# wzx99/DCFP

Measured on AMD Instinct MI355X. Metric: training images/sec at 1024x2048 DeepLabv3-R101, higher is better.
Workload: dtype f32

## Files before the change

dcfp_amd/csrc/conv_igemm.hip:

```cpp
#include "common.h"
#include <string.h>
#include <stdio.h>
#include <stdlib.h>

namespace {

int check_desc(const DcfpConvDesc* d) {
    if (!d) return DCFP_E_BADDESC;
    if (d->N <= 0 || d->Cin <= 0 || d->Cout <= 0 || d->H <= 0 || d->W <= 0 || d->stride <= 0 ||
        d->dil <= 0 || d->pad < 0)
        return DCFP_E_BADDESC;
    if (d->KH != d->KW || (d->KH != 1 && d->KH != 3)) return DCFP_E_UNSUPPORTED;
    const int ho = (d->H + 2 * d->pad - d->dil * (d->KH - 1) - 1) / d->stride + 1;
    const int wo = (d->W + 2 * d->pad - d->dil * (d->KW - 1) - 1) / d->stride + 1;
    if (ho != d->Hout || wo != d->Wout || ho <= 0 || wo <= 0) return DCFP_E_BADDESC;
    if ((d->x_pitch != 0 && (d->x_pitch < d->W || (d->x_pitch & 3))) ||
        (d->dy_pitch != 0 && (d->dy_pitch < d->Wout || (d->dy_pitch & 3))))
        return DCFP_E_BADDESC;
    if ((long long)d->Cin * d->H * (d->x_pitch ? d->x_pitch : d->W) >= (1LL << 29) ||
        (long long)d->Cout * d->Hout * (d->dy_pitch ? d->dy_pitch : d->Wout) >= (1LL << 29) ||
        (long long)d->Cout * d->Cin * d->KH * d->KW >= (1LL << 29))
        return DCFP_E_UNSUPPORTED;
    return DCFP_OK;
}
// ... 12 lines not shown
                    const float* bias, float* out, long long out_nstride, int N, int M, int Ck, int T,
                    int Hi, int Wi, int Ho, int Wo, int sn, int sd, int off0, int offstep,
                    int accumulate, void* workspace, size_t workspace_bytes, hipStream_t stream,
                    const float* scale = nullptr, const float* shift = nullptr,
                    const float* residual = nullptr, int relu = 0, float* stat_part = nullptr, int wp_valid = 0,
                    int in_pitch = 0, long long wp_nstride = 0, const float* fan_src = nullptr,
                    const unsigned long long* fan_mask = nullptr, const Igemm2Red* red = nullptr);
bool dcfp_wino_ok(int N, int H, int W, int d, int M, int Ck);
size_t dcfp_wino_workspace_bytes(int N, int H, int W, int d, int M, int Ck);
double dcfp_wino_exec_fraction(int N, int H, int W, int d, int M, int Ck);
int dcfp_wino_run(const float* in, long long in_nstride, int in_pitch, const float* w, int sAm, int sAc, int flip,
                  float* out, long long out_nstride, int N, int M, int Ck, int H, int W, int d, int accumulate,
                  void* workspace, size_t workspace_bytes, hipStream_t stream, float* xform_out = nullptr,
                  float* stat_part = nullptr, const float* scale = nullptr, const float* shift = nullptr,
                  const float* residual = nullptr, int relu = 0, int wp_valid = 0);
long long dcfp_wino_stat_slots(int N, int H, int W, int d);
bool dcfp_stem_shape(const DcfpConvDesc* d);
int dcfp_stem_fwd(const DcfpConvDesc* d, const float* x, const float* w, const float* bias, float* y, long long y_nstride,
                  hipStream_t stream, float* stat_part = nullptr);
long long dcfp_stem_stat_slots(const DcfpConvDesc* d, const float* y, long long y_nstride);
bool dcfp_gemv_shape(const DcfpConvDesc* d);
int dcfp_gemv_fwd(const DcfpConvDesc* d, const float* x, const float* w, const float* bias, float* y, long long y_nstride,
                  hipStream_t stream);
int dcfp_gemv_dgrad(const DcfpConvDesc* d, const float* dy, long long dy_nstride, const float* w, float* dx, int accumulate,
                    hipStream_t stream);
bool dcfp_wino_fused_ok(int N, int H, int W, int d, int M, int Ck, long long in_nstride, int pitch);
size_t dcfp_wino_fused_workspace_bytes(int N, int H, int W, int d, int M, int Ck);
void dcfp_wino_fused_pads(int N, int H, int W, int d, int M, int Ck, int* CkP, int* Mpad);
size_t dcfp_wino_xform_bytes(int N, int H, int W, int d, int C);
bool dcfp_wgrad_is_winograd(const DcfpConvDesc* d);
bool dcfp_wgrad_wants_xform(const DcfpConvDesc* d);
long long dcfp_igemm2_stat_slots(int M, int P, int N, long long out_nstride, const float* out);
bool dcfp_igemm2_dma_shape(int T, int M, int Ck, int P, long long px, int sn, int sd, int off0, int HiWi, int Wo);
bool dcfp_igemm2_persist();
void dcfp_igemm2_wp_layout(int T, int M, int Ck, int P, long long px, int sn, int sd, int off0, int offstep, int HiWi,
                           int Wo, bool pitched, int sAm, int sAc, DcfpWpEntry* e);
bool dcfp_igemm2_use_dma8(int T, int M, int P, long long px, int sn, int sd, int off0, int offstep, int HiWi,
                          int Wo, bool pitched);
int dcfp_igemm2_permute_multi(const DcfpWpEntry* table, int n, long long total_blocks, hipStream_t stream);


size_t dcfp_igemm3_workspace_bytes(int T, int M, int Ck);
int dcfp_igemm3_run(const float* in, long long in_nstride, const float* w, int sAm, int sAc,
                    const float* bias, float* out, long long out_nstride, int N, int M, int Ck, int T,
                    int Hi, int Wi, int Ho, int Wo, int off0, int offstep, int accumulate,
                    void* workspace, size_t workspace_bytes, hipStream_t stream,
                    const float* scale = nullptr, const float* shift = nullptr,
                    const float* residual = nullptr, int relu = 0, int wp_valid = 0);
int dcfp_igemm2_cfg_id(int M, long long px, int sd);
static bool math_bf16x3() {
    static const bool v = [] { const char* e = getenv("DCFP_CONV_MATH"); return e && !strcmp(e, "bf16x3"); }();
    return v;
}
static bool igemm3_ok(int M, long long px, int sn, int sd) {
    return math_bf16x3() && sn == 1 && sd == 1 && dcfp_igemm2_cfg_id(M, px, sd) == 4;
}

static int wino_kind(const DcfpConvDesc* d, int pass) {
    static const int mode = [] { const char* e = getenv("DCFP_CONV_WINOGRAD"); return e ? atoi(e) : 1; }();
    if (mode == 0) return 0;
    if (d->KH != 3 || d->KW != 3 || d->stride != 1 || d->pad != d->dil || d->Hout != d->H || d->Wout != d->W)
        return 0;
    if (math_bf16x3()) return 0;
    const bool fwd = pass == DCFP_CONV_FWD;
    const int M = fwd ? d->Cout : d->Cin, Ck = fwd ? d->Cin : d->Cout;
    const int sp = fwd ? d->x_pitch : d->dy_pitch;
// ... 66 lines not shown
        const long long px = (long long)d->N * d->H * d->W;
        b2 = dcfp_igemm2_workspace_bytes(T, d->Cin, d->Cout, px, d->stride);
        if (igemm3_ok(d->Cin, px, 1, d->stride)) b3 = dcfp_igemm3_workspace_bytes(T, d->Cin, d->Cout);
    }
    return b2 > b3 ? b2 : b3;
}

extern "C" int dcfp_conv2d_kernel_name(const DcfpConvDesc* d, int pass, char* buf, int buf_len) {
    int rc = check_desc(d);
    if (rc) return rc;
    if (!buf || buf_len <= 0) return DCFP_E_BADDESC;
    if (dcfp_gemv_shape(d)) return snprintf(buf, buf_len, "gemv_1x1_map_kernel");
    if (pass == DCFP_CONV_WGRAD) return dcfp_wgrad_kernel_name(d, buf, buf_len);
    if (pass == DCFP_CONV_FWD && dcfp_stem_shape(d)) return snprintf(buf, buf_len, "stem_fwd_kernel");
    if (const int wk = wino_kind(d, pass))
        return wk == 1 ? snprintf(buf, buf_len, "winograd_f2x2_3x3 (igemm2_dma1p_kernel<false,true>)")
                       : snprintf(buf, buf_len, "winograd_f2x2_3x3 fused (wino_fused_kernel)");
    const int M = pass == DCFP_CONV_FWD ? d->Cout : d->Cin;
    const long long px = pass == DCFP_CONV_FWD ? (long long)d->N * d->Hout * d->Wout : (long long)d->N * d->H * d->W;
    const int sd = pass == DCFP_CONV_FWD ? 1 : d->stride;
    if (igemm3_ok(M, px, pass == DCFP_CONV_FWD ? d->stride : 1, sd))
        return snprintf(buf, buf_len, "igemm3_kernel<%d>", d->KH * d->KW);
    const int P = pass == DCFP_CONV_FWD ? d->Hout * d->Wout : d->H * d->W;
    const int HiWi = pass == DCFP_CONV_FWD ? d->H * d->W : d->Hout * d->Wout;
    const int Ck = pass == DCFP_CONV_FWD ? d->Cin : d->Cout;
    {
        const int sp = pass == DCFP_CONV_FWD ? d->x_pitch : d->dy_pitch;
        const bool pitched = sp && sp != (pass == DCFP_CONV_FWD ? d->W : d->Wout);
        if (dcfp_igemm2_use_dma8(d->KH * d->KW, M, P, px, pass == DCFP_CONV_FWD ? d->stride : 1, sd,
                                 pass == DCFP_CONV_FWD ? -d->pad : d->pad, pass == DCFP_CONV_FWD ? d->dil : -d->dil,
                                 HiWi, pass == DCFP_CONV_FWD ? d->Wout : d->W, pitched))
            return snprintf(buf, buf_len, "igemm2_dma8_kernel<%d>", d->KH * d->KW);
    }
    if (dcfp_igemm2_dma_shape(d->KH * d->KW, M, Ck, P, px, pass == DCFP_CONV_FWD ? d->stride : 1, sd, d->pad, HiWi,
                              pass == DCFP_CONV_FWD ? d->Wout : d->W)) {
        if (d->KH == 1 && dcfp_igemm2_persist()) return snprintf(buf, buf_len, "igemm2_dma1p_kernel");
        const int src_pitch = pass == DCFP_CONV_FWD ? d->x_pitch : d->dy_pitch;
        const bool pitched = src_pitch && src_pitch != (pass == DCFP_CONV_FWD ? d->W : d->Wout);
        return snprintf(buf, buf_len, "igemm2_dma_kernel<%d,%s>", d->KH * d->KW,
                        (d->KH == 3 && ((d->pad | d->dil) & 3) != 0 && !pitched) ? "true" : "false");
    }
    return snprintf(buf, buf_len, "igemm2_kernel<%d,%s>", d->KH * d->KW, dcfp_igemm2_cfg_args(M, px, sd));
}

extern "C" double dcfp_conv2d_executed_fraction(const DcfpConvDesc* d, int pass) {
    if (check_desc(d) != DCFP_OK) return 1.0;
    if (pass == DCFP_CONV_WGRAD) return dcfp_wgrad_exec_fraction(d);
    const bool fwd = pass == DCFP_CONV_FWD;
    if (wino_pass(d, pass))
        return fwd ? dcfp_wino_exec_fraction(d->N, d->H, d->W, d->dil, d->Cout, d->Cin)
                   : dcfp_wino_exec_fraction(d->N, d->H, d->W, d->dil, d->Cin, d->Cout);
    const int M = fwd ? d->Cout : d->Cin;
    const long long px = fwd ? (long long)d->N * d->Hout * d->Wout : (long long)d->N * d->H * d->W;
    if (igemm3_ok(M, px, fwd ? d->stride : 1, fwd ? 1 : d->stride)) return 1.0;
    const int sp = fwd ? d->x_pitch : d->dy_pitch;
    const bool pitched = sp && sp != (fwd ? d->W : d->Wout);
    return fwd ? dcfp_igemm2_exec_fraction(d->KH * d->KW, d->Cout, d->Cin, d->N, d->H, d->W, d->Hout, d->Wout, d->stride, 1,
                                           -d->pad, d->dil, pitched)
               : dcfp_igemm2_exec_fraction(d->KH * d->KW, d->Cin, d->Cout, d->N, d->Hout, d->Wout, d->H, d->W, 1, d->stride,
                                           d->pad, -d->dil, pitched);
}

extern "C" int64_t dcfp_conv2d_fwd_stat_slots(const DcfpConvDesc* d, const float* y, int64_t y_nstride);

extern "C" size_t dcfp_conv2d_xform_bytes(const DcfpConvDesc* d) {
    if (check_desc(d) != DCFP_OK) return 0;
// ... 240 lines not shown
```

dcfp_amd/csrc/conv_igemm2.hip:

```cpp
#include "igemm2_common.h"
#include <queue>
#include <vector>
#include <stdio.h>
#include <stdlib.h>

namespace {

__device__ __forceinline__ int wp_row(int m, int perm8) {
    if (!perm8) return m;
    const int j = m & 255;
    return (m & ~255) + 32 * (j & 7) + (j >> 3);
}

__global__ void __launch_bounds__(256)
permute_weights_kernel(const float* __restrict__ w, float* __restrict__ wp, int T, int Ck, int CkP,
                       int M, int Mpad, int sAm, int sAc, int perm8) {
    const long long total = (long long)T * CkP * Mpad;
    for (long long i = (long long)blockIdx.x * 256 + threadIdx.x; i < total;
         i += (long long)gridDim.x * 256) {
        const int m = wp_row((int)(i % Mpad), perm8);
        const long long r = i / Mpad;
        const int c = (int)(r % CkP);
        const int t = (int)(r / CkP);
        float v = 0.f;
// ... 5 lines not shown
constexpr int kWpBlockElems = DCFP_WP_BLOCK_ELEMS;
__global__ void __launch_bounds__(256)
permute_weights_multi_kernel(const DcfpWpEntry* __restrict__ table, int n) {
    const long long blk = blockIdx.x;
    int lo = 0, hi = n - 1;
    while (lo < hi) {
        const int mid = (lo + hi + 1) >> 1;
        if (table[mid].first_block <= blk) lo = mid; else hi = mid - 1;
    }
    const DcfpWpEntry e = table[lo];
    const long long base = (blk - e.first_block) * kWpBlockElems;
    if (e.perm8 >= 2) {
        const long long pairs = (long long)e.CkP * e.Mpad;
#pragma unroll 1
        for (int u = 0; u < kWpBlockElems / 256; ++u) {
            const long long i = base + u * 256 + threadIdx.x;
            if (i >= pairs) return;
            wino_filter2_pair(e.w, e.sAm, e.sAc, e.perm8 == 3, e.M, e.Ck, e.Mpad, i, e.wp);
        }
        return;
    }
    const long long total = (long long)e.T * e.CkP * e.Mpad;
#pragma unroll
    for (int u = 0; u < kWpBlockElems / 256; ++u) {
        const long long i = base + u * 256 + threadIdx.x;
        if (i >= total) return;
        const int m = wp_row((int)(i % e.Mpad), e.perm8);
        const long long r = i / e.Mpad;
        const int c = (int)(r % e.CkP);
        const int t = (int)(r / e.CkP);
        float v = 0.f;
        if (m < e.M && c < e.Ck) v = e.w[(long long)m * e.sAm + (long long)c * e.sAc + t];
        e.wp[i] = v;
    }
}

__device__ __forceinline__ float half_xor(float v, int mask) {
    switch (mask) {
        case 1: return __builtin_bit_cast(float, __builtin_amdgcn_ds_swizzle(__builtin_bit_cast(int, v), (1 << 10) | 0x1f));
        case 2: return __builtin_bit_cast(float, __builtin_amdgcn_ds_swizzle(__builtin_bit_cast(int, v), (2 << 10) | 0x1f));
        case 4: return __builtin_bit_cast(float, __builtin_amdgcn_ds_swizzle(__builtin_bit_cast(int, v), (4 << 10) | 0x1f));
        case 8: return __builtin_bit_cast(float, __builtin_amdgcn_ds_swizzle(__builtin_bit_cast(int, v), (8 << 10) | 0x1f));
        default: return __builtin_bit_cast(float, __builtin_amdgcn_ds_swizzle(__builtin_bit_cast(int, v), (16 << 10) | 0x1f));
    }
}

template <int TAPS, int TM, int TN, int WM, int WN, bool SD, bool ACC, int KB = 16>
__global__ void __launch_bounds__(64 * WM * WN, (TM * TN <= 8 && WM * WN == 4 && !ACC) ? 2 : 1)
igemm2_kernel(const Igemm2Params p) {
    constexpr int BK = KB;
    constexpr int NPART = BK / 4;
    constexpr int BM = WM * TM * 32, BN = WN * TN * 32, NT = 64 * WM * WN;
    constexpr int AX = BM / 4;
    constexpr int AROWS = (NT / AX) < BK ? (NT / AX) : BK;
    constexpr int APASS = BK / AROWS;
    constexpr int TX = BN / 4, TY = NT / TX, RPT = BK / TY;
    static_assert(APASS >= 1 && APASS * AROWS == BK, "A loader shape");
    static_assert(TY >= 1 && RPT >= 1 && TY * RPT == BK, "B loader shape");

    extern __shared__ __attribute__((aligned(16))) float smem[];
    float* As = smem;
    float* Bs = smem + 2 * BK * BM;

    const int group = 8 * p.tiles_m;
    const int g = blockIdx.x / group, local = blockIdx.x - g * group;
    const int nt = g * 8 + (local & 7);
    const int mt = local >> 3;
    if (nt >= p.tiles_n_total) return;
    const int img = nt / p.tiles_per_img;
    const int ti_img = nt - img * p.tiles_per_img;
    const int phase = SD ? (p.zfold ? p.zfold - 1 : ti_img / p.tiles_per_phase) : 0;
    const int ph_h = SD ? phase / p.sd : 0, ph_w = SD ? phase - ph_h * p.sd : 0;
    const int p0 = (SD && !p.zfold ? ti_img - phase * p.tiles_per_phase : ti_img) * BN;
    const int m0 = mt * BM;

    const int tid = threadIdx.x;
// ... 886 lines not shown
        p.tile2d = (!d8 && fits && !pitched && ((off0 | offstep) & 3) != 0 && Ho == Hi && Wo == Wi) ? t2d : 0;
    }
    if (pick_tapskip(p, 256) == 0) return 1.0;
    long long live = 0;
    for (int ti = 0; ti < p.tiles_per_img; ++ti) live += tile_live_rows(p, ti);
    return (double)live / (3.0 * p.tiles_per_img);
}

void dcfp_igemm2_wp_layout(int T, int M, int Ck, int P, long long px, int sn, int sd, int off0, int offstep, int HiWi,
                           int Wo, bool pitched, int sAm, int sAc, DcfpWpEntry* e) {
    const TileCfg c = pick_cfg(M, px, sd);
    const bool d8 = dcfp_igemm2_use_dma8(T, M, P, px, sn, sd, off0, offstep, HiWi, Wo, pitched);
    e->T = T; e->Ck = Ck; e->CkP = round_up(Ck, ck_pad()); e->M = M; e->Mpad = round_up(M, d8 ? 256 : c.bm);
    e->sAm = sAm; e->sAc = sAc; e->perm8 = d8 ? 1 : 0;
}

int dcfp_igemm2_permute_multi(const DcfpWpEntry* table, int n, long long total_blocks, hipStream_t stream) {
    hipLaunchKernelGGL(permute_weights_multi_kernel, dim3((unsigned)total_blocks), dim3(256), 0, stream, table, n);
    DCFP_RETURN_LAUNCH();
}

bool dcfp_igemm2_persist() {
    static const bool persist = [] { const char* e = getenv("DCFP_IGEMM_PERSIST"); return !e || atoi(e) != 0; }();
    return persist;
}

bool dcfp_igemm2_dma_shape(int T, int M, int Ck, int P, long long px, int sn, int sd, int off0, int HiWi, int Wo) {
    static const bool dma = [] { const char* e = getenv("DCFP_IGEMM_DMA"); return !e || atoi(e) != 0; }();
    static const bool dma9 = [] { const char* e = getenv("DCFP_IGEMM_DMA9"); return !e || atoi(e) != 0; }();
    if (!dma || pick_cfg(M, px, sd).id != 4 || sn != 1 || sd != 1 || HiWi != P || Wo % 4 != 0) return false;
    return T == 1 ? off0 == 0 : dma9;
}

int dcfp_igemm2_run(const float* in, long long in_nstride, const float* w, int sAm, int sAc,
                    const float* bias, float* out, long long out_nstride, int N, int M, int Ck, int T,
                    int Hi, int Wi, int Ho, int Wo, int sn, int sd, int off0, int offstep,
                    int accumulate, void* workspace, size_t workspace_bytes, hipStream_t stream,
                    const float* scale, const float* shift, const float* residual, int relu,
                    float* stat_part, int wp_valid, int in_pitch, long long wp_nstride, const float* fan_src,
                    const unsigned long long* fan_mask, const Igemm2Red* red) {
    const long long px = (long long)N * Ho * Wo;
    const TileCfg c = pick_cfg(M, px, sd);
    Igemm2Params p;
    p.stat_part = stat_part;
    p.wp_nstride = wp_nstride;
    p.fan_src = fan_src; p.fan_mask = fan_mask;
    p.red_x = red ? red->x : nullptr; p.red_mask = red ? red->mask : nullptr;
    p.red_mean = red ? red->mean : nullptr; p.red_part = red ? red->part : nullptr;
    if (red && !fan_src) return DCFP_E_BADDESC;
    p.in = in; p.bias = bias; p.out = out;
    p.scale = scale; p.shift = shift; p.residual = residual; p.relu = relu;
    p.in_nstride = in_nstride; p.out_nstride = out_nstride;
    p.N = N; p.M = M; p.Ck = Ck; p.CkP = round_up(Ck, ck_pad()); p.Mpad = round_up(M, c.bm);
    const bool plain = !scale && !relu && !stat_part;
    const bool d8 = plain && !wp_nstride && !fan_src && dcfp_igemm2_use_dma8(T, M, Ho * Wo, px, sn, sd, off0, offstep, Hi * Wi, Wo,
                                                                 in_pitch > 0 && in_pitch != Wi);
    if (d8) p.Mpad = round_up(M, 256);
    p.Hi = Hi; p.Wi = Wi; p.Ho = Ho; p.Wo = Wo; p.P = Ho * Wo;
    p.in_pitch = in_pitch > 0 ? in_pitch : Wi;
    const bool pitched = p.in_pitch != Wi;
    if (pitched) {
        const int reach = off0 < 0 ? -off0 : off0;
        if (T != 9 || p.in_pitch < Wi + reach || off0 + 2 * offstep != -off0 || (p.in_pitch & 3) ||
            (!d8 && (bias || !dcfp_igemm2_dma_shape(T, M, Ck, Ho * Wo, px, sn, sd, off0, Hi * Wi, Wo))) || scale || relu)
            return DCFP_E_UNSUPPORTED;
        if (!d8 && stat_part && dcfp_igemm2_use_dma8(T, M, Ho * Wo, px, sn, sd, off0, offstep, Hi * Wi, Wo, true))
            return DCFP_E_UNSUPPORTED;
    }
    {
        static const int t2d = [] { const char* e = getenv("DCFP_IGEMM_2D"); return e ? atoi(e) : 5; }();
        const bool fits = (t2d == 4 || t2d == 5) && Hi % (256 >> t2d) == 0 && Wi % (1 << t2d) == 0;
        p.tile2d = (fits && !pitched && T == 9 && ((off0 | offstep) & 3) != 0 && Ho == Hi && Wo == Wi) ? t2d : 0;
    }
    p.tapskip = 0;
    {
        static const int nt = [] { const char* e = getenv("DCFP_IGEMM_NT"); return e ? atoi(e) : 0; }();
        p.nt_store = nt;
    }
    p.tiles_per_img = (p.P + (d8 ? 256 : c.bn) - 1) / (d8 ? 256 : c.bn);
    p.Hc = p.Wc = p.tiles_per_phase = p.zfold = 0;
    if (sd > 1) {
        p.Hc = (Ho + sd - 1) / sd; p.Wc = (Wo + sd - 1) / sd;
        p.tiles_per_phase = (p.Hc * p.Wc + c.bn - 1) / c.bn;
        p.tiles_per_img = sd * sd * p.tiles_per_phase;
        if (T == 1) {
            const int ph = ((-off0) % sd + sd) % sd;
            p.zfold = ph * sd + ph + 1;
            p.tiles_per_img = p.tiles_per_phase;
        }
    }
    p.tiles_n_total = p.tiles_per_img * N;
    p.tiles_m = p.Mpad / (d8 ? 256 : c.bm);
    p.sn = sn; p.sd = sd; p.off0 = off0; p.offstep = offstep;
    p.accumulate = accumulate;
    p.vec_store = (p.P % 4 == 0) && (out_nstride % 4 == 0) && dcfp_aligned16(out);
    if (T == 9 && sd == 1 && sn == 1) p.tapskip = pick_tapskip(p, d8 ? 256 : c.bn);
    const size_t need = (size_t)T * p.CkP * p.Mpad * sizeof(float);
    if (!workspace || workspace_bytes < need || !dcfp_aligned16(workspace)) return DCFP_E_WORKSPACE;
    float* wp = static_cast<float*>(workspace);
    p.wp = wp;
    if (!wp_valid) {
        const long long total = (long long)T * p.CkP * p.Mpad;
        long long b = (total + 255) / 256;
        if (b > 2048) b = 2048;
        hipLaunchKernelGGL(permute_weights_kernel, dim3((unsigned)b), dim3(256), 0, stream, w, wp, T,
                           Ck, p.CkP, M, p.Mpad, sAm, sAc, d8 ? 1 : 0);
    }
    if (d8) {
        if (!p.vec_store || wp_nstride || fan_src) return DCFP_E_UNSUPPORTED;
        return dcfp_igemm2n_launch(p, T, stream);
    }
    if (dcfp_igemm2_dma_shape(T, M, Ck, p.P, px, sn, sd, off0, Hi * Wi, Wo) && p.vec_store && !bias && !scale &&
        !relu && !(stat_part && accumulate)) {
        const long long groups = ((long long)p.tiles_n_total + 7) / 8;
        const long long blocks = groups * 8 * p.tiles_m;
        const size_t lds = stat_part ? (size_t)4 * 64 * 33 * 8 : (size_t)2 * BK * 512 * sizeof(float);
        auto launch = [&](auto kern) -> int {
            hipError_t e = hipFuncSetAttribute(reinterpret_cast<const void*>(kern),
                                               hipFuncAttributeMaxDynamicSharedMemorySize, (int)lds);
            if (e != hipSuccess) return (int)e;
            hipLaunchKernelGGL(kern, dim3((unsigned)blocks), dim3(256), lds, stream, p);
            DCFP_RETURN_LAUNCH();
        };
        if (T == 1) {
            if (fan_src && (M % 256 != 0 || p.P % 256 != 0 || !dcfp_igemm2_persist())) return DCFP_E_UNSUPPORTED;
            if (dcfp_igemm2_persist()) return dcfp_igemm2p_launch(p, stream);
            if (wp_nstride) return DCFP_E_UNSUPPORTED;
            return accumulate ? launch(igemm2_dma_kernel<1, false, true>) : launch(igemm2_dma_kernel<1, false, false>);
        }
        if (((off0 | offstep) & 3) == 0 || pitched)
            return accumulate ? launch(igemm2_dma_kernel<9, false, true>) : launch(igemm2_dma_kernel<9, false, false>);
        return accumulate ? launch(igemm2_dma_kernel<9, true, true>) : launch(igemm2_dma_kernel<9, true, false>);
    }
    if (wp_nstride || fan_src) return DCFP_E_UNSUPPORTED;
    return T == 1 ? launch_taps<1>(p, c.id, stream) : launch_taps<9>(p, c.id, stream);
}

int dcfp_igemm2_ck_pad() { return ck_pad(); }
```

dcfp_amd/csrc/conv_igemm2p.hip:

```cpp
#include "igemm2_common.h"
#include <stdlib.h>

namespace {

typedef unsigned u32x4 __attribute__((vector_size(16)));
typedef __attribute__((address_space(3))) void* lds_ptr;

__device__ __forceinline__ u32x4 make_desc(const void* base, unsigned bytes) {
    const unsigned long long a = (unsigned long long)base;
    u32x4 d = {(unsigned)a, (unsigned)(a >> 32) & 0xffffu, bytes, 0x00020000u};
    return d;
}

constexpr int kStatFloats = 4 * 64 * 33 * 2;
constexpr int kStatFloats2 = 4 * 32 * 32 * 2;

template <bool ACC, bool WPI = false, int TM_ = 4, bool FAN = false, bool RED = false>
__global__ void __launch_bounds__(256, TM_ == 2 ? 2 : 1) igemm2_dma1p_kernel(const Igemm2Params p, int total_tiles, int dbg) {
    constexpr int TM = TM_, TN = 4, WN = 2, BM = 64 * TM_, BN = 256;
    extern __shared__ __attribute__((aligned(16))) float smem[];
    float* As = smem;
    float* Bs = smem + 2 * BK * BM;
    float* Ss = smem + 2 * BK * (BM + BN);
    const int tid = threadIdx.x;
    const int lane = tid & 63, wid = tid >> 6;
    const int wm = wid / WN, wn = wid - wm * WN;
    const int l31 = lane & 31, lhi = lane >> 5;
    const int HiWi = p.Hi * p.Wi;
    const int group = 8 * p.tiles_m;
    const int nk = p.CkP / BK;

    const int wid_s = __builtin_amdgcn_readfirstlane(wid);
    const unsigned lane16 = lane * 16u;
    const unsigned a2_voff = (unsigned)((lane >> 5) * p.Mpad) * 4u + (unsigned)(lane & 31) * 16u;
    const u32x4 a_desc = make_desc(p.wp, 0x7ffffffcu);
    const unsigned lds_a0 = (unsigned)(size_t)(lds_ptr)As, lds_b0 = (unsigned)(size_t)(lds_ptr)Bs;

    auto decode = [&](int t, int& nt, int& mt) {
        const int g = t / group, local = t - g * group;
        nt = g * 8 + (local & 7);
        mt = local >> 3;
    };
    auto next_valid = [&](int t) {
        while (t < total_tiles) {
            int nt, mt;
            decode(t, nt, mt);
            if (nt < p.tiles_n_total) break;
            t += gridDim.x;
        }
        return t;
    };

    int ld_tile = next_valid(blockIdx.x), ld_cb = 0;
    unsigned ld_boff4 = 0;
    unsigned a_run = 0, b_run = 0;
    u32x4 ld_bdesc = a_desc;
    const unsigned a_row = (unsigned)p.Mpad * 4u, b_row = (unsigned)HiWi * 4u;
    const unsigned a_kstep = (unsigned)(BK * p.Mpad) * 4u, b_kstep = (unsigned)(BK * HiWi) * 4u;
    const unsigned lds_a_w = __builtin_amdgcn_readfirstlane(lds_a0 + (unsigned)(4 * wid_s * BM) * 4u);
    const unsigned lds_b_w = __builtin_amdgcn_readfirstlane(lds_b0 + (unsigned)(4 * wid_s * BN) * 4u);
    auto ld_set_tile = [&]() {
        int nt, mt;
        decode(ld_tile, nt, mt);
        const int img = nt / p.tiles_per_img;
        const int p0 = (nt - img * p.tiles_per_img) * BN;
        a_run = __builtin_amdgcn_readfirstlane((unsigned)(mt * BM + (WPI ? img * (int)p.wp_nstride : 0)) * 4u +
                                               (unsigned)(4 * wid_s) * a_row);
        b_run = __builtin_amdgcn_readfirstlane((unsigned)(4 * wid_s) * b_row);
        ld_bdesc = make_desc(p.in + (long long)img * p.in_nstride, (unsigned)(p.Ck * HiWi) * 4u);
        const int pp = p0 + 4 * lane;
        ld_boff4 = pp < p.P ? (unsigned)pp * 4u : kOob;
    };
    auto issue_piece = [&](unsigned abuf, unsigned bbuf, auto piece_) {
        constexpr int piece = decltype(piece_)::value;
        constexpr int q = piece >> 1;
        if constexpr ((piece & 1) == 0) {
            if constexpr (TM == 4) {
                const unsigned a_s = a_run + (unsigned)q * a_row;
                const unsigned av = lane16;
                const u32x4 ad = a_desc;
                asm volatile("s_add_i32 m0, %0, %4\n\ts_nop 0\n\tbuffer_load_dwordx4 %1, %2, %3 offen lds"
                             :: "s"(abuf), "v"(av), "s"(ad), "s"(a_s), "i"(q * BM * 4) : "memory", "m0", "scc");
            } else if constexpr (q < 2) {
                const unsigned a_s = a_run + (unsigned)(2 * q) * a_row;
                const unsigned av = a2_voff;
                const u32x4 ad = a_desc;
                asm volatile("s_add_i32 m0, %0, %4\n\ts_nop 0\n\tbuffer_load_dwordx4 %1, %2, %3 offen lds"
                             :: "s"(abuf), "v"(av), "s"(ad), "s"(a_s), "i"(2 * q * BM * 4) : "memory", "m0", "scc");
            }
        } else {
            const unsigned b_cb = b_run + (unsigned)q * b_row;
            const unsigned b_s = 0;
            const unsigned bv = ld_boff4 + b_cb;
            const u32x4 bd = ld_bdesc;
            asm volatile("s_add_i32 m0, %0, %4\n\ts_nop 0\n\tbuffer_load_dwordx4 %1, %2, %3 offen lds"
                         :: "s"(bbuf), "v"(bv), "s"(bd), "s"(b_s), "i"(q * BN * 4) : "memory", "m0", "scc");
        }
    };
    auto ld_advance = [&]() {
        a_run += a_kstep;
        b_run += b_kstep;
        if (++ld_cb == nk) {
            ld_cb = 0;
            ld_tile = next_valid(ld_tile + gridDim.x);
            if (ld_tile < total_tiles) ld_set_tile();
        }
    };
    auto issue = [&](int buf) {
        const unsigned abuf = lds_a_w + (buf ? (unsigned)(BK * BM) * 4u : 0u), bbuf = lds_b_w + (buf ? (unsigned)(BK * BN) * 4u : 0u);
        static_for<0, 8>([&](auto piece_) { issue_piece(abuf, bbuf, piece_); });
        ld_advance();
    };
    auto retire = [&]() {
        asm volatile("s_waitcnt vmcnt(0) lgkmcnt(0)" ::: "memory");
        __builtin_amdgcn_s_barrier();
    };

    int tile = ld_tile;
    if (tile >= total_tiles) return;
#ifdef DCFP_P_DEBUG
    if (dbg & 0xff00) {
// ... 47 lines not shown
                    });
                });
                __builtin_amdgcn_sched_barrier(0);
            });
            retire();
            cur ^= 1;
        }

        float* o_img = p.out + (long long)img * p.out_nstride;
#ifdef DCFP_P_DEBUG
        if (dbg & 1) {
            if (acc[0][0][0] == 123.456f) o_img[0] = 1.f;
            tile = next_tile;
            continue;
        }
#endif
        if (m0 + BM > p.M || p0 + BN > p.P) {
            int pix = p0 + wn * (TN * 32) + TN * l31;
            asm volatile("" : "+v"(pix));
#pragma unroll
            for (int i = 0; i < TM; ++i) {
#pragma unroll
                for (int r = 0; r < 16; ++r) {
                    const int row = (r & 3) + 8 * (r >> 2) + 4 * lhi;
                    const int m = m0 + wm * (TM * 32) + TM * row + i;
                    if (m >= p.M || pix >= p.P) continue;
                    float* dst = o_img + (long long)m * p.P + pix;
                    f32x4 v = {acc[i][0][r], acc[i][1][r], acc[i][2][r], acc[i][3][r]};
                    if constexpr (ACC) v += *reinterpret_cast<const f32x4*>(dst);
                    *reinterpret_cast<f32x4*>(dst) = v;
                }
            }
        } else {
            if constexpr (!ACC && TM == 4) {
                if (p.stat_part) {
                    typedef float f32x2 __attribute__((ext_vector_type(2)));
                    f32x2* st = reinterpret_cast<f32x2*>(Ss) + wid * (64 * 33);
                    float* sp = p.stat_part + ((long long)(nt * WN + wn) * p.M + m0 + wm * (TM * 32)) * 2;
                    static_for<0, 2>([&](auto h_) {
                        constexpr int half = decltype(h_)::value;
                        static_for<0, 2>([&](auto ii_) {
                            constexpr int ii = decltype(ii_)::value;
                            constexpr int i = 2 * half + ii;
                            static_for<0, 16>([&](auto r_) {
                                constexpr int r = decltype(r_)::value;
                                const float a0 = acc[i][0][r], a1 = acc[i][1][r], a2 = acc[i][2][r], a3 = acc[i][3][r];
                                const float s4 = (a0 + a1) + (a2 + a3);
                                const float mu = 0.25f * s4;
                                const float d0 = a0 - mu, d1 = a1 - mu, d2 = a2 - mu, d3 = a3 - mu;
                                f32x2 v = {s4, (d0 * d0 + d1 * d1) + (d2 * d2 + d3 * d3)};
                                st[(lhi * 32 + ii * 16 + r) * 33 + l31] = v;
                            });
                        });
                        float S = 0.f, M2 = 0.f;
#pragma unroll
                        for (int k = 0; k < 32; ++k) {
                            const f32x2 v = st[lane * 33 + k];
                            S += v.x; M2 += v.y;
                        }
                        const float mean = S * (1.0f / 128.0f);
                        __builtin_amdgcn_sched_barrier(0);
#pragma unroll
                        for (int k = 0; k < 32; ++k) {
                            const float d = 0.25f * st[lane * 33 + k].x - mean;
                            M2 += 4.0f * d * d;
                        }
                        const int rr = lane & 15;
                        const int row = 16 * (lane >> 5) + 4 * (rr & 3) + 32 * (rr >> 2) + 2 * half + ((lane >> 4) & 1);
                        sp[row * 2] = mean;
                        sp[row * 2 + 1] = M2;
                    });
                }
            }
            if constexpr (!ACC && TM == 2 && !FAN) {
                if (p.stat_part) {
                    typedef float f32x2 __attribute__((ext_vector_type(2)));
                    f32x2* st = reinterpret_cast<f32x2*>(Ss) + wid * (32 * 32);
                    float* sp = p.stat_part + ((long long)(nt * WN + wn) * p.M + m0 + wm * (TM * 32)) * 2;
                    static_for<0, 2>([&](auto i_) {
                        constexpr int i = decltype(i_)::value;
                        static_for<0, 16>([&](auto r_) {
                            constexpr int r = decltype(r_)::value;
                            const float a0 = acc[i][0][r], a1 = acc[i][1][r], a2 = acc[i][2][r], a3 = acc[i][3][r];
                            const float s4 = (a0 + a1) + (a2 + a3);
                            const float mu = 0.25f * s4;
                            const float d0 = a0 - mu, d1 = a1 - mu, d2 = a2 - mu, d3 = a3 - mu;
                            f32x2 v = {s4, (d0 * d0 + d1 * d1) + (d2 * d2 + d3 * d3)};
                            const int row = lhi * 16 + r;
                            st[row * 32 + ((l31 + row) & 31)] = v;
                        });
                        const int rw = lane & 31;
                        float S = 0.f, M2 = 0.f;
#pragma unroll
                        for (int k = 0; k < 32; ++k) {
                            const f32x2 v = st[rw * 32 + ((k + rw) & 31)];
                            S += v.x; M2 += v.y;
                        }
                        const float mean = S * (1.0f / 128.0f);
                        __builtin_amdgcn_sched_barrier(0);
#pragma unroll
                        for (int k = 0; k < 32; ++k) {
                            const float d = 0.25f * st[rw * 32 + ((k + rw) & 31)].x - mean;
                            M2 += 4.0f * d * d;
                        }
                        if (lane < 32) {
                            const int rr = lane & 15;
                            const int row = 2 * ((rr & 3) + 8 * (rr >> 2) + 4 * (lane >> 4)) + i;
// ... 115 lines not shown
                    __builtin_amdgcn_sched_barrier(0);
                }
                static_for<0, 16>([&](auto r_) {
                    constexpr int r = decltype(r_)::value;
                    constexpr int row = TM * ((r & 3) + 8 * (r >> 2)) + i;
                    f32x4 v = {acc[i][0][r], acc[i][1][r], acc[i][2][r], acc[i][3][r]};
                    if constexpr (ACC) v += old[r];
                    typedef __attribute__((__vector_size__(4 * sizeof(unsigned)))) unsigned u4;
                    if (ACC || p.nt_store == 0)
                        __builtin_amdgcn_raw_buffer_store_b128(__builtin_bit_cast(u4, v),
                            o_rsrc, voff + (unsigned)row * P4, 0, 0);
                    else if (p.nt_store == 1)
                        __builtin_amdgcn_raw_buffer_store_b128(__builtin_bit_cast(u4, v), o_rsrc, voff + (unsigned)row * P4, 0, 2);
                    else
                        __builtin_amdgcn_raw_buffer_store_b128(__builtin_bit_cast(u4, v), o_rsrc, voff + (unsigned)row * P4, 0, 18);
                });
                if constexpr (ACC) __builtin_amdgcn_sched_barrier(0);
            });
        }
        tile = next_tile;
    }
}

}

static int p128_mode() {
    static const int p128 = [] { const char* e = getenv("DCFP_IGEMM_P128"); return e ? atoi(e) : 2; }();
    return p128;
}
bool dcfp_igemm2p_fan_red_ok(int Mpad, int CkP) {
    return Mpad % 256 == 0 && (p128_mode() == 2 || (p128_mode() == 1 && CkP <= 256));
}

int dcfp_igemm2p_launch(const Igemm2Params& p, hipStream_t stream) {
    static int cus = 0;
    if (cus == 0) {
        int dev = 0, v = 0;
        if (hipGetDevice(&dev) == hipSuccess &&
            hipDeviceGetAttribute(&v, hipDeviceAttributeMultiprocessorCount, dev) == hipSuccess && v > 0)
            cus = v;
        else
            cus = 256;
    }
    const int p128 = p128_mode();
    static const int half_stats = [] { const char* e = getenv("DCFP_IGEMM_P128_STATS"); return e ? atoi(e) : 2; }();
    const bool k_ok = p128 == 2 || (p128 == 1 && p.CkP <= 256);
    const bool half = p.Mpad % 256 == 0 &&
                      (p.stat_part ? (!p.accumulate && !p.fan_src && !p.wp_nstride && (half_stats == 2 || (half_stats == 1 && k_ok)))
                                   : k_ok);
    Igemm2Params q = p;
    if (half) q.tiles_m = p.tiles_m * 2;
    const long long groups = ((long long)p.tiles_n_total + 7) / 8;
    const long long total = groups * 8 * q.tiles_m;
    if (total > 0x7fffffffLL) return DCFP_E_UNSUPPORTED;
    const long long slots = half ? 2LL * cus : cus;
    long long blocks = total < slots ? total : slots;
    int dbg = 0;
#ifdef DCFP_P_DEBUG
    if (const char* e = getenv("DCFP_DBG_P_BLOCKS")) blocks = atoll(e) < blocks ? atoll(e) : blocks;
    if (const char* e = getenv("DCFP_DBG_P")) dbg = atoi(e);
#endif
    blocks = blocks / 8 * 8;
    if (blocks < 8) blocks = total < 8 ? total : 8;
    const size_t lds = (size_t)(2 * BK * (half ? 384 : 512) + (p.stat_part ? (half ? kStatFloats2 : kStatFloats) : 0)) * sizeof(float);
    auto launch = [&](auto kern) -> int {
        hipError_t e = hipFuncSetAttribute(reinterpret_cast<const void*>(kern),
                                           hipFuncAttributeMaxDynamicSharedMemorySize, (int)lds);
        if (e != hipSuccess) return (int)e;
        hipLaunchKernelGGL(kern, dim3((unsigned)blocks), dim3(256), lds, stream, q, (int)total, dbg);
        DCFP_RETURN_LAUNCH();
    };
    if (p.wp_nstride) {
        if (p.accumulate) return DCFP_E_UNSUPPORTED;
        return half ? launch(igemm2_dma1p_kernel<false, true, 2>) : launch(igemm2_dma1p_kernel<false, true>);
    }
    if (p.fan_src) {
// ... 12 lines not shown
```

dcfp_amd/csrc/igemm2_common.h:

```cpp
#pragma once
#include "common.h"
#include <type_traits>

struct Igemm2Params {
    const float* in;
    const float* wp;
    const float* bias;
    const float* scale;
    const float* shift;
    const float* residual;
    int relu;
    float* out;
    long long in_nstride, out_nstride;
    int N, M, Mpad, Ck, CkP;
    int Hi, Wi, Ho, Wo, P, tiles_per_img, tiles_n_total, tiles_m;
    int sn, sd, off0, offstep;
    int accumulate, vec_store;
    int tile2d;
    int Hc, Wc, tiles_per_phase;
    int in_pitch;
    int zfold;
    const float* fan_src;
    const unsigned long long* fan_mask;
    long long wp_nstride;
// ... 26 lines not shown
                                                  int Mpad, long long idx, float* __restrict__ Ug) {
    const int mblocks = Mpad / 64;
    const int c = (int)(idx / Mpad), m = (int)(idx - (long long)c * Mpad);
    float g[9];
    if (m < M && c < Ck) {
        const float* src = w + (long long)m * sAm + (long long)c * sAc;
#pragma unroll
        for (int t = 0; t < 9; ++t) g[t] = src[flip ? 8 - t : t];
    } else {
#pragma unroll
        for (int t = 0; t < 9; ++t) g[t] = 0.f;
    }
    float r[4][3];
#pragma unroll
    for (int k = 0; k < 3; ++k) {
        const float g0 = g[k], g1 = g[3 + k], g2 = g[6 + k];
        r[0][k] = g0;
        r[1][k] = 0.5f * ((g0 + g2) + g1);
        r[2][k] = 0.5f * ((g0 + g2) - g1);
        r[3][k] = g2;
    }
    const int cb = c >> 3, cl = c & 7, mb = m >> 6, ml = m & 63;
    float* dst = Ug + ((((long long)(cb * mblocks + mb) * 16) * 2 + (ml >> 5)) * 64 + (cl & 1) * 32 + (ml & 31)) * 4 + (cl >> 1);
#pragma unroll
    for (int i = 0; i < 4; ++i) {
        const float a = r[i][0], b = r[i][1], cc = r[i][2];
        dst[(4 * i + 0) * 512] = a;
        dst[(4 * i + 1) * 512] = 0.5f * ((a + cc) + b);
        dst[(4 * i + 2) * 512] = 0.5f * ((a + cc) - b);
        dst[(4 * i + 3) * 512] = cc;
    }
}

template <int T>
struct Frag;
template <>
struct Frag<4> {
    static __device__ __forceinline__ void ld(const float* p, float (&f)[4]) {
        const float4 v = *reinterpret_cast<const float4*>(p);
        f[0] = v.x; f[1] = v.y; f[2] = v.z; f[3] = v.w;
    }
};
template <>
struct Frag<2> {
    static __device__ __forceinline__ void ld(const float* p, float (&f)[2]) {
        const float2 v = *reinterpret_cast<const float2*>(p);
        f[0] = v.x; f[1] = v.y;
    }
};
template <>
struct Frag<1> {
    static __device__ __forceinline__ void ld(const float* p, float (&f)[1]) { f[0] = p[0]; }
};

}
```

Before: 12.28.

## Route narrow-M 1x1 convs to persistent DMA kernel with 64/128-row tiles

Adds a 'narrow' path that sends stride-1, unpadded 1x1 convolutions with M<=128 (cfg ids 1 or 2) to the persistent igemm2_dma1p kernel, instantiated with TM=1 or TM=2 and BN=256, in place of the generic igemm2 kernel. It adds a TM=1 weight-load path, a butterfly (ds_swizzle) reduction that produces per-tile BN mean/M2 statistics without going through LDS, and a launcher that chooses 2 or 3 blocks per CU. The aim is to bring the async LDS-DMA pipeline and persistent scheduling to small-M 1x1 layers. The risk is lower occupancy or less reuse than the tuned generic configs, plus a different summation order in the statistics.

```diff
diff --git a/dcfp_amd/csrc/conv_igemm.hip b/dcfp_amd/csrc/conv_igemm.hip
--- a/dcfp_amd/csrc/conv_igemm.hip
+++ b/dcfp_amd/csrc/conv_igemm.hip
@@ -68,6 +68,7 @@
 bool dcfp_wgrad_wants_xform(const DcfpConvDesc* d);
 long long dcfp_igemm2_stat_slots(int M, int P, int N, long long out_nstride, const float* out);
 bool dcfp_igemm2_dma_shape(int T, int M, int Ck, int P, long long px, int sn, int sd, int off0, int HiWi, int Wo);
+bool dcfp_igemm2_narrow(int T, int M, int P, long long px, int sn, int sd, int off0, int HiWi, int Wo);
 bool dcfp_igemm2_persist();
 void dcfp_igemm2_wp_layout(int T, int M, int Ck, int P, long long px, int sn, int sd, int off0, int offstep, int HiWi,
                            int Wo, bool pitched, int sAm, int sAc, DcfpWpEntry* e);
@@ -200,6 +201,9 @@
                                  HiWi, pass == DCFP_CONV_FWD ? d->Wout : d->W, pitched))
             return snprintf(buf, buf_len, "igemm2_dma8_kernel<%d>", d->KH * d->KW);
     }
+    if (dcfp_igemm2_narrow(d->KH * d->KW, M, P, px, pass == DCFP_CONV_FWD ? d->stride : 1, sd, d->pad, HiWi,
+                           pass == DCFP_CONV_FWD ? d->Wout : d->W))
+        return snprintf(buf, buf_len, "igemm2_dma1p_kernel (%d x 256)", dcfp_igemm2_cfg_id(M, px, sd) == 1 ? 64 : 128);
     if (dcfp_igemm2_dma_shape(d->KH * d->KW, M, Ck, P, px, pass == DCFP_CONV_FWD ? d->stride : 1, sd, d->pad, HiWi,
                               pass == DCFP_CONV_FWD ? d->Wout : d->W)) {
         if (d->KH == 1 && dcfp_igemm2_persist()) return snprintf(buf, buf_len, "igemm2_dma1p_kernel");
diff --git a/dcfp_amd/csrc/conv_igemm2.hip b/dcfp_amd/csrc/conv_igemm2.hip
--- a/dcfp_amd/csrc/conv_igemm2.hip
+++ b/dcfp_amd/csrc/conv_igemm2.hip
@@ -61,16 +61,6 @@
         float v = 0.f;
         if (m < e.M && c < e.Ck) v = e.w[(long long)m * e.sAm + (long long)c * e.sAc + t];
         e.wp[i] = v;
-    }
-}
-
-__device__ __forceinline__ float half_xor(float v, int mask) {
-    switch (mask) {
-        case 1: return __builtin_bit_cast(float, __builtin_amdgcn_ds_swizzle(__builtin_bit_cast(int, v), (1 << 10) | 0x1f));
-        case 2: return __builtin_bit_cast(float, __builtin_amdgcn_ds_swizzle(__builtin_bit_cast(int, v), (2 << 10) | 0x1f));
-        case 4: return __builtin_bit_cast(float, __builtin_amdgcn_ds_swizzle(__builtin_bit_cast(int, v), (4 << 10) | 0x1f));
-        case 8: return __builtin_bit_cast(float, __builtin_amdgcn_ds_swizzle(__builtin_bit_cast(int, v), (8 << 10) | 0x1f));
-        default: return __builtin_bit_cast(float, __builtin_amdgcn_ds_swizzle(__builtin_bit_cast(int, v), (16 << 10) | 0x1f));
     }
 }
 
@@ -1023,6 +1013,16 @@
     return T == 1 ? off0 == 0 : dma9;
 }
 
+bool dcfp_igemm2_narrow(int T, int M, int P, long long px, int sn, int sd, int off0, int HiWi, int Wo) {
+    static const bool on = [] { const char* e = getenv("DCFP_IGEMM_NARROW"); return !e || atoi(e) != 0; }();
+    static const bool dma = [] { const char* e = getenv("DCFP_IGEMM_DMA"); return !e || atoi(e) != 0; }();
+    if (!on || !dma || !dcfp_igemm2_persist() || deep_k() || T != 1 || off0 != 0 || sn != 1 || sd != 1 || HiWi != P ||
+        Wo % 4 != 0 || M > 128)
+        return false;
+    const int id = pick_cfg(M, px, sd).id;
+    return id == 1 || id == 2;
+}
+
 int dcfp_igemm2_run(const float* in, long long in_nstride, const float* w, int sAm, int sAc,
                     const float* bias, float* out, long long out_nstride, int N, int M, int Ck, int T,
                     int Hi, int Wi, int Ho, int Wo, int sn, int sd, int off0, int offstep,
@@ -1047,6 +1047,9 @@
     const bool d8 = plain && !wp_nstride && !fan_src && dcfp_igemm2_use_dma8(T, M, Ho * Wo, px, sn, sd, off0, offstep, Hi * Wi, Wo,
                                                                  in_pitch > 0 && in_pitch != Wi);
     if (d8) p.Mpad = round_up(M, 256);
+    const bool narrow = !d8 && dcfp_igemm2_narrow(T, M, Ho * Wo, px, sn, sd, off0, Hi * Wi, Wo) && !wp_nstride && !fan_src &&
+                        !bias && !scale && !relu && !(stat_part && accumulate) && (Ho * Wo) % 4 == 0 && out_nstride % 4 == 0 &&
+                        dcfp_aligned16(out);
     p.Hi = Hi; p.Wi = Wi; p.Ho = Ho; p.Wo = Wo; p.P = Ho * Wo;
     p.in_pitch = in_pitch > 0 ? in_pitch : Wi;
     const bool pitched = p.in_pitch != Wi;
@@ -1068,7 +1071,8 @@
         static const int nt = [] { const char* e = getenv("DCFP_IGEMM_NT"); return e ? atoi(e) : 0; }();
         p.nt_store = nt;
     }
-    p.tiles_per_img = (p.P + (d8 ? 256 : c.bn) - 1) / (d8 ? 256 : c.bn);
+    const int bn = d8 || narrow ? 256 : c.bn;
+    p.tiles_per_img = (p.P + bn - 1) / bn;
     p.Hc = p.Wc = p.tiles_per_phase = p.zfold = 0;
     if (sd > 1) {
         p.Hc = (Ho + sd - 1) / sd; p.Wc = (Wo + sd - 1) / sd;
@@ -1124,6 +1128,7 @@
         return accumulate ? launch(igemm2_dma_kernel<9, true, true>) : launch(igemm2_dma_kernel<9, true, false>);
     }
     if (wp_nstride || fan_src) return DCFP_E_UNSUPPORTED;
+    if (narrow) return dcfp_igemm2p_launch(p, stream);
     return T == 1 ? launch_taps<1>(p, c.id, stream) : launch_taps<9>(p, c.id, stream);
 }
 
diff --git a/dcfp_amd/csrc/conv_igemm2p.hip b/dcfp_amd/csrc/conv_igemm2p.hip
--- a/dcfp_amd/csrc/conv_igemm2p.hip
+++ b/dcfp_amd/csrc/conv_igemm2p.hip
@@ -15,8 +15,8 @@
 constexpr int kStatFloats = 4 * 64 * 33 * 2;
 constexpr int kStatFloats2 = 4 * 32 * 32 * 2;
 
-template <bool ACC, bool WPI = false, int TM_ = 4, bool FAN = false, bool RED = false>
-__global__ void __launch_bounds__(256, TM_ == 2 ? 2 : 1) igemm2_dma1p_kernel(const Igemm2Params p, int total_tiles, int dbg) {
+template <bool ACC, bool WPI = false, int TM_ = 4, bool FAN = false, bool RED = false, bool BFLY = false>
+__global__ void __launch_bounds__(256, TM_ == 4 ? 1 : (TM_ == 2 ? 2 : 3)) igemm2_dma1p_kernel(const Igemm2Params p, int total_tiles, int dbg) {
     constexpr int TM = TM_, TN = 4, WN = 2, BM = 64 * TM_, BN = 256;
     extern __shared__ __attribute__((aligned(16))) float smem[];
     float* As = smem;
@@ -32,7 +32,8 @@
 
     const int wid_s = __builtin_amdgcn_readfirstlane(wid);
     const unsigned lane16 = lane * 16u;
-    const unsigned a2_voff = (unsigned)((lane >> 5) * p.Mpad) * 4u + (unsigned)(lane & 31) * 16u;
+    const unsigned an_voff = TM == 1 ? (unsigned)((lane >> 4) * p.Mpad) * 4u + (unsigned)(lane & 15) * 16u
+                                     : (unsigned)((lane >> 5) * p.Mpad) * 4u + (unsigned)(lane & 31) * 16u;
     const u32x4 a_desc = make_desc(p.wp, 0x7ffffffcu);
     const unsigned lds_a0 = (unsigned)(size_t)(lds_ptr)As, lds_b0 = (unsigned)(size_t)(lds_ptr)Bs;
 
@@ -81,12 +82,18 @@
                 const u32x4 ad = a_desc;
                 asm volatile("s_add_i32 m0, %0, %4\n\ts_nop 0\n\tbuffer_load_dwordx4 %1, %2, %3 offen lds"
                              :: "s"(abuf), "v"(av), "s"(ad), "s"(a_s), "i"(q * BM * 4) : "memory", "m0", "scc");
-            } else if constexpr (q < 2) {
+            } else if constexpr (TM == 2 && q < 2) {
                 const unsigned a_s = a_run + (unsigned)(2 * q) * a_row;
-                const unsigned av = a2_voff;
+                const unsigned av = an_voff;
                 const u32x4 ad = a_desc;
                 asm volatile("s_add_i32 m0, %0, %4\n\ts_nop 0\n\tbuffer_load_dwordx4 %1, %2, %3 offen lds"
                              :: "s"(abuf), "v"(av), "s"(ad), "s"(a_s), "i"(2 * q * BM * 4) : "memory", "m0", "scc");
+            } else if constexpr (TM == 1 && q == 0) {
+                const unsigned a_s = a_run;
+                const unsigned av = an_voff;
+                const u32x4 ad = a_desc;
+                asm volatile("s_add_i32 m0, %0, %4\n\ts_nop 0\n\tbuffer_load_dwordx4 %1, %2, %3 offen lds"
+                             :: "s"(abuf), "v"(av), "s"(ad), "s"(a_s), "i"(0) : "memory", "m0", "scc");
             }
         } else {
             const unsigned b_cb = b_run + (unsigned)q * b_row;
@@ -200,7 +207,7 @@
                 }
             }
         } else {
-            if constexpr (!ACC && TM == 4) {
+            if constexpr (!ACC && TM == 4 && !BFLY) {
                 if (p.stat_part) {
                     typedef float f32x2 __attribute__((ext_vector_type(2)));
                     f32x2* st = reinterpret_cast<f32x2*>(Ss) + wid * (64 * 33);
@@ -240,7 +247,44 @@
                     });
                 }
             }
-            if constexpr (!ACC && TM == 2 && !FAN) {
+            if constexpr (!ACC && BFLY) {
+                if (p.stat_part) {
+                    float* sp = p.stat_part +
+                                ((long long)(nt * WN + wn) * p.M + m0 + wm * (TM * 32) + TM * 4 * lhi) * 2;
+                    static_for<0, TM>([&](auto i_) {
+                        constexpr int i = decltype(i_)::value;
+                        float sm[16], q[16];
+                        static_for<0, 16>([&](auto r_) {
+                            constexpr int r = decltype(r_)::value;
+                            sm[r] = (acc[i][0][r] + acc[i][1][r]) + (acc[i][2][r] + acc[i][3][r]);
+                        });
+                        static_for<0, 5>([&](auto st_) {
+                            constexpr int mask = 1 << decltype(st_)::value;
+                            static_for<0, 16>([&](auto r_) { constexpr int r = decltype(r_)::value; sm[r] += half_xor(sm[r], mask); });
+                        });
+                        static_for<0, 16>([&](auto r_) {
+                            constexpr int r = decltype(r_)::value;
+                            sm[r] *= (1.0f / 128.0f);
+                            const float d0 = acc[i][0][r] - sm[r], d1 = acc[i][1][r] - sm[r];
+                            const float d2 = acc[i][2][r] - sm[r], d3 = acc[i][3][r] - sm[r];
+                            q[r] = (d0 * d0 + d1 * d1) + (d2 * d2 + d3 * d3);
+                        });
+                        static_for<0, 5>([&](auto st_) {
+                            constexpr int mask = 1 << decltype(st_)::value;
+                            static_for<0, 16>([&](auto r_) { constexpr int r = decltype(r_)::value; q[r] += half_xor(q[r], mask); });
+                        });
+                        if (l31 == 0) {
+                            static_for<0, 16>([&](auto r_) {
+                                constexpr int r = decltype(r_)::value;
+                                constexpr int row = TM * ((r & 3) + 8 * (r >> 2)) + i;
+                                sp[row * 2] = sm[r]; sp[row * 2 + 1] = q[r];
+                            });
+                        }
+                        __builtin_amdgcn_sched_barrier(0);
+                    });
+                }
+            }
+            if constexpr (!ACC && TM == 2 && !FAN && !BFLY) {
                 if (p.stat_part) {
                     typedef float f32x2 __attribute__((ext_vector_type(2)));
                     f32x2* st = reinterpret_cast<f32x2*>(Ss) + wid * (32 * 32);
@@ -422,6 +466,33 @@
     return Mpad % 256 == 0 && (p128_mode() == 2 || (p128_mode() == 1 && CkP <= 256));
 }
 
+static int narrow_launch(const Igemm2Params& p, int bm, int cus, hipStream_t stream) {
+    if ((bm != 128 && bm != 64) || p.wp_nstride || p.fan_src || (p.accumulate && p.stat_part)) return DCFP_E_UNSUPPORTED;
+    const long long groups = ((long long)p.tiles_n_total + 7) / 8;
+    const long long total = groups * 8 * p.tiles_m;
+    if (total > 0x7fffffffLL) return DCFP_E_UNSUPPORTED;
+    int per_cu = 2;
+    if (bm == 64) {
+        auto busiest = [&](long long k) { return (total + k * cus - 1) / (k * cus) * k; };
+        per_cu = busiest(3) <= busiest(2) ? 3 : 2;
+    }
+    const long long slots = (long long)per_cu * cus;
+    long long blocks = total < slots ? total : slots;
+    blocks = blocks / 8 * 8;
+    if (blocks < 8) blocks = total < 8 ? total : 8;
+    const size_t lds = (size_t)2 * BK * (bm + 256) * sizeof(float);
+    auto launch = [&](auto kern) -> int {
+        hipError_t e = hipFuncSetAttribute(reinterpret_cast<const void*>(kern),
+                                           hipFuncAttributeMaxDynamicSharedMemorySize, (int)lds);
+        if (e != hipSuccess) return (int)e;
+        hipLaunchKernelGGL(kern, dim3((unsigned)blocks), dim3(256), lds, stream, p, (int)total, 0);
+        DCFP_RETURN_LAUNCH();
+    };
+    if (bm == 128)
+        return p.accumulate ? launch(igemm2_dma1p_kernel<true, false, 2>) : launch(igemm2_dma1p_kernel<false, false, 2, false, false, true>);
+    return p.accumulate ? launch(igemm2_dma1p_kernel<true, false, 1>) : launch(igemm2_dma1p_kernel<false, false, 1, false, false, true>);
+}
+
 int dcfp_igemm2p_launch(const Igemm2Params& p, hipStream_t stream) {
     static int cus = 0;
     if (cus == 0) {
@@ -432,6 +503,9 @@
         else
             cus = 256;
     }
+    if (p.tiles_m <= 0 || p.Mpad % p.tiles_m != 0) return DCFP_E_BADDESC;
+    const int bm = p.Mpad / p.tiles_m;
+    if (bm != 256) return narrow_launch(p, bm, cus, stream);
     const int p128 = p128_mode();
     static const int half_stats = [] { const char* e = getenv("DCFP_IGEMM_P128_STATS"); return e ? atoi(e) : 2; }();
     const bool k_ok = p128 == 2 || (p128 == 1 && p.CkP <= 256);
diff --git a/dcfp_amd/csrc/igemm2_common.h b/dcfp_amd/csrc/igemm2_common.h
--- a/dcfp_amd/csrc/igemm2_common.h
+++ b/dcfp_amd/csrc/igemm2_common.h
@@ -82,6 +82,16 @@
     }
 }
 
+__device__ __forceinline__ float half_xor(float v, int mask) {
+    switch (mask) {
+        case 1: return __builtin_bit_cast(float, __builtin_amdgcn_ds_swizzle(__builtin_bit_cast(int, v), (1 << 10) | 0x1f));
+        case 2: return __builtin_bit_cast(float, __builtin_amdgcn_ds_swizzle(__builtin_bit_cast(int, v), (2 << 10) | 0x1f));
+        case 4: return __builtin_bit_cast(float, __builtin_amdgcn_ds_swizzle(__builtin_bit_cast(int, v), (4 << 10) | 0x1f));
+        case 8: return __builtin_bit_cast(float, __builtin_amdgcn_ds_swizzle(__builtin_bit_cast(int, v), (8 << 10) | 0x1f));
+        default: return __builtin_bit_cast(float, __builtin_amdgcn_ds_swizzle(__builtin_bit_cast(int, v), (16 << 10) | 0x1f));
+    }
+}
+
 template <int T>
 struct Frag;
 template <>
```

After: 12.30, median of 6. About the same (+0.2%).
